# myshell-ai/OpenVoice

Measured on NVIDIA H100. Metric: audio_seconds_per_second, higher is better.
Workload: dtype f32 (3xFP16 split-precision tensor-core convs with fp32 accumulation, fp32 FFMA elsewhere)

## Files before the change

### include/ovc.h

```cpp
#ifndef OVC_B200_H
#define OVC_B200_H

#include <stddef.h>
#include <stdint.h>

#ifdef __cplusplus
extern "C" {
#endif

#define OVC_ABI_VERSION 17

#if defined(__GNUC__)
#define OVC_API __attribute__((visibility("default")))
#else
#define OVC_API
#endif

enum {
  OVC_OK = 0,
  OVC_ERR_INVALID = -1,
  OVC_ERR_CUDA = -2,
  OVC_ERR_STATE = -3,
  OVC_ERR_MISSING = -4,
  OVC_ERR_NOMEM = -5
};
// ... 154 lines not shown
                                      float* d_stats, int32_t* d_cum, float* d_g, int64_t* d_y_lengths, void* stream);
OVC_API int ovc_tts_decode_windows_tokens(ovc_ctx* ctx, const float* stats, const int32_t* cum, const float* g,
                                          const int64_t* y_lengths, int N, int T, const int64_t* row, const int64_t* frame0,
                                          const int64_t* len, int W, int Wmax, const uint64_t* seed, const int64_t* stream,
                                          const float* noise_scale, float* o, float* z_p, void* cuda_stream);

OVC_API int ovc_set_precision(ovc_ctx* ctx, int mode);

#define OVC_OPT_TTS_SIMPLE 2
#define OVC_OPT_GRAPH 3
#define OVC_OPT_PDL 5
#define OVC_OPT_BRANCHES 7
#define OVC_OPT_PAIR 8
#define OVC_OPT_PAIR_OCC 9
#define OVC_OPT_STAGED_EPI 10
OVC_API int ovc_set_option(ovc_ctx* ctx, int key, int value);

OVC_API int ovc_last_launch_count(const ovc_ctx* ctx);

OVC_API int ovc_graph_replays(const ovc_ctx* ctx);

OVC_API int ovc_profile_enable(ovc_ctx* ctx, int enable);
OVC_API int ovc_profile_read(ovc_ctx* ctx, double* ms, int64_t* launches, double* flops, double* bytes);
OVC_API int ovc_profile_detail(ovc_ctx* ctx, int max, char* names, double* ms, double* flops, double* bytes,
                               int* family);

OVC_API int ovc_debug_enable(ovc_ctx* ctx, int enable);
OVC_API int ovc_debug_fetch(ovc_ctx* ctx, const char* name, float* host_out, size_t max_floats,
                    int64_t* shape4 );

// ... 5 lines not shown
```

### openvoice_b200/_native.py

```python
from __future__ import annotations

import ctypes as C
import os
from typing import Dict, Iterable, Optional, Tuple

_HERE = os.path.dirname(os.path.abspath(__file__))
LIB_PATH = os.path.join(_HERE, "libovc_b200.so")

ABI_VERSION = 17
EXPORTS = (
    "ovc_abi_version", "ovc_last_error", "ovc_create", "ovc_destroy", "ovc_load_tensor",
    "ovc_finalize_weights", "ovc_workspace_floats", "ovc_voice_conversion", "ovc_last_launch_count",
    "ovc_profile_enable", "ovc_profile_read", "ovc_profile_detail", "ovc_debug_enable", "ovc_debug_fetch",
    "ovc_spectrogram", "ovc_convert_waveform", "ovc_set_precision", "ovc_reference_encoder",
    "ovc_tts_info", "ovc_tts_encode", "ovc_tts_decode", "ovc_set_option", "ovc_graph_replays",
    "ovc_reference_encoder_ragged", "ovc_resample", "ovc_resample_span", "ovc_voice_conversion_items",
    "ovc_convert_waveform_items", "ovc_tts_encode_items", "ovc_tts_decode_items", "ovc_philox_normals",
    "ovc_tts_encode_state", "ovc_tts_decode_windows", "ovc_spectrogram_ring", "ovc_splice",
    "ovc_tts_encode_state_rows", "ovc_tts_state_rows", "ovc_resample_plan", "ovc_resample_rings",
    "ovc_voice_conversion_frames", "ovc_convert_waveform_frames", "ovc_tone_track_expand",
    "ovc_tts_encode_g", "ovc_tts_encode_state_tokens", "ovc_tts_decode_windows_tokens", "ovc_tts_encode_state_rows_tokens",
    "ovc_tts_state_rows_tokens", "ovc_reference_encoder_stream", "ovc_reference_encoder_stream_state_floats",
    "ovc_generate_frames",
)
# ... 259 lines not shown
            _check(self.lib, rc, f"ovc_load_tensor({k})")
            (ignored if rc == 1 else used).append(k)
        self.finalized = False
        return used, ignored

    def finalize(self):
        _check(self.lib, self.lib.ovc_finalize_weights(self.handle), "ovc_finalize_weights")
        self.finalized = True

    def set_precision(self, mode: str):
        m = PRECISIONS[mode]
        _check(self.lib, self.lib.ovc_set_precision(self.handle, m), "ovc_set_precision")
        self.precision = mode

    def set_option(self, key: str, value: int):
        k = {"tts_simple": 2, "graph": 3, "pdl": 5, "branches": 7, "pair": 8, "pair_occ": 9, "staged_epi": 10}[key]
        _check(self.lib, self.lib.ovc_set_option(self.handle, k, int(value)), "ovc_set_option")

    def voice_conversion(self, spec, lengths, g_src, g_tgt, noise=None, tau: float = 0.3, seed: int = 0,
                         ragged: bool = False, latents: bool = True, stream=None, items: Optional[dict] = None, out=None):
        import torch
        assert spec.is_cuda and spec.dtype == torch.float32 and spec.is_contiguous()
        assert lengths.is_cuda and lengths.dtype == torch.int64 and lengths.is_contiguous()
        B, S, T = spec.shape
        gs, fs = se_arg(g_src, B, self.hp.gin_channels, T, "g_src")
        gt, ft = se_arg(g_tgt, B, self.hp.gin_channels, T, "g_tgt")
        if noise is not None:
            noise = noise.contiguous().float()
            assert tuple(noise.shape) == (B, self.hp.inter_channels, T)
        hop = self.hp.hop_length
        if out is not None:
# ... 486 lines not shown
```

### openvoice_b200/csrc/ovc_lib.cu

```cuda
#include <cuda_runtime.h>

#include <algorithm>
#include <cmath>
#include <cstdarg>
#include <cstdio>
#include <cstdlib>
#include <cstring>
#include <map>
#include <string>
#include <vector>

#include "../../include/ovc.h"
#include "ovc_convpack.h"
#include "ovc_small.cuh"
#include "ovc_tcconv.cuh"
#include "ovc_tts.cuh"
#include "ovc_refenc.cuh"
#include "ovc_resample.cuh"
#include "ovc_splice.h"
#include "ovc_variants.h"

namespace ovc {

static thread_local std::string g_err;
// ... 135 lines not shown
  WNLayers flow_wn[4];
  ConvLayer dec_pre, dec_ups[4];
  ConvLayer rb_c1[12][3], rb_c2[12][3];
  TcLayer tc_c1[12][3], tc_c2[12][3], tc_ups[4], tc_pre;
  float* d_tcw = nullptr;
  std::vector<float> h_tcw;
  int precision = 0;
  bool tts_simple = false;
  bool use_graph = true;
  int use_pdl = 2;
  bool use_branches = true;
  int par_frames = 512;
  bool use_pair = true;
  bool use_pair_occ = true;
  bool use_staged_epi = true;
  bool pair_occ2_ok[TCN_N_OCC2] = {};
  cudaStream_t br_stream[2] = {nullptr, nullptr};
  cudaEvent_t br_ev[4] = {nullptr, nullptr, nullptr, nullptr};
  size_t post_w_off = 0;
  size_t cond_w_off = 0, cond_b_off = 0;
  int* d_cond_wrow = nullptr;
  int* d_cond_sel = nullptr;
  int cond_rows_out = 0;
  int cond_off_enc = 0, cond_off_fsrc = 0, cond_off_ftgt = 0, cond_off_dec = 0;
  int cond_off_enc_tc = 0, cond_off_fsrc_tc = 0, cond_off_ftgt_tc = 0;
  int* d_cond_cols[2][3] = {};
  int cond_pf_cols[2][3] = {};
  int cond_pf_off[2][3][4] = {};

  float2* d_tw = nullptr;
// ... 427 lines not shown
  if (c->d_w) { cudaFree(c->d_w); c->d_w = nullptr; }
  c->w_floats = c->h_w.size();
  CK(cudaMalloc(&c->d_w, c->w_floats * sizeof(float)));
  CK(cudaMemcpy(c->d_w, c->h_w.data(), c->w_floats * sizeof(float), cudaMemcpyHostToDevice));
  if (c->d_tcw) { cudaFree(c->d_tcw); c->d_tcw = nullptr; }
  CK(cudaMalloc(&c->d_tcw, c->h_tcw.size() * sizeof(float)));
  CK(cudaMemcpy(c->d_tcw, c->h_tcw.data(), c->h_tcw.size() * sizeof(float), cudaMemcpyHostToDevice));
  c->h_tcw.clear();
  c->h_tcw.shrink_to_fit();
  for (int TN : {128, 64, 32})
    for (bool staged : {false, true}) {
      const TcKernel k = tc_conv_kernel(TN, staged), p = tc_pair_kernel(TN, TcPairOcc(), staged);
      CK(cudaFuncSetAttribute(k.fn, cudaFuncAttributeMaxDynamicSharedMemorySize, (int)k.smem));
      CK(cudaFuncSetAttribute(p.fn, cudaFuncAttributeMaxDynamicSharedMemorySize, (int)p.smem));
    }
  for (int i = 0; i < TCN_N_OCC2; ++i) {
    const TcKernel k = tc_pair_kernel(kTcPairOcc2[i].C, kTcPairOcc2[i].o);
    CK(cudaFuncSetAttribute(k.fn, cudaFuncAttributeMaxDynamicSharedMemorySize, (int)k.smem));
    int blocks = 0;
    CK(cudaOccupancyMaxActiveBlocksPerMultiprocessor(&blocks, k.fn, k.threads, k.smem));
    c->pair_occ2_ok[i] = blocks >= 2;
    if (blocks < 2)
      fprintf(stderr, "ovc: the C = %d conv-pair kernel with %d operand buffer(s) fits %d CTA(s) per SM, not 2; its pairs run "
              "one CTA per SM\n", kTcPairOcc2[i].C, kTcPairOcc2[i].o.nabuf, blocks);
  }
  if (c->d_cond_wrow) cudaFree(c->d_cond_wrow);
  if (c->d_cond_sel) cudaFree(c->d_cond_sel);
  CK(cudaMalloc(&c->d_cond_wrow, wrow.size() * sizeof(int)));
  CK(cudaMalloc(&c->d_cond_sel, sel.size() * sizeof(int)));
  CK(cudaMemcpy(c->d_cond_wrow, wrow.data(), wrow.size() * sizeof(int), cudaMemcpyHostToDevice));
// ... 135 lines not shown
  CK(cudaEventRecord(c->ev[c->ev_used], r.st));
  return OVC_OK;
}
static int prof_end(Run& r, int variant, int family, double flops, double bytes, int tag = 0) {
  ovc_ctx* c = r.c;
  if (!c->prof) return OVC_OK;
  CK(cudaEventRecord(c->ev[c->ev_used + 1], r.st));
  c->ev_used += 2;
  c->ev_flops.push_back(flops);
  c->ev_bytes.push_back(bytes);
  c->ev_variant.push_back(variant);
  c->ev_family.push_back(family);
  c->ev_tag.push_back(tag);
  return OVC_OK;
}
enum { V_TCPAIR128 = -14, V_TCPAIR64 = -12, V_TCPAIR32 = -13, V_TC128 = -1, V_TC64 = -2, V_TC32 = -3, V_TRANSPOSE = -4, V_TTS_DENSE = -5, V_TTS_LN = -6, V_TTS_SCORES = -7,
       V_TTS_ATTN = -8, V_TTS_DW = -9, V_TTS_SPLINE = -10, V_TTS_MISC = -11 };
static const char* variant_name(int v) {
  if (v >= 0) return kInfo[v].name;
  switch (v) {
    case V_TCPAIR128: return "PAIR_N128";
    case V_TCPAIR64: return "PAIR_N64";
    case V_TCPAIR32: return "PAIR_N32";
    case V_TC128: return "TC3_N128";
    case V_TC64: return "TC3_N64";
    case V_TC32: return "TC3_N32";
    case V_TTS_DENSE: return "TTS_DENSE32";
    case V_TTS_LN: return "TTS_LAYERNORM";
    case V_TTS_SCORES: return "TTS_SCORES";
    case V_TTS_ATTN: return "TTS_ATTN_OUT";
    case V_TTS_DW: return "TTS_DWCONV";
    case V_TTS_SPLINE: return "TTS_SPLINE";
    case V_TTS_MISC: return "TTS_MISC";
    default: return "TRANSPOSE";
  }
}

// ... 58 lines not shown
}

static int launch_pair(Run& r, const TcLayer& T1, const TcLayer& T2, const float* x, float* y, int t_len, int mul, float slope,
                       float scale, int accumulate) {
  TcConvArgs a{};
  const int C = T1.TN;
  a.x = x; a.x_bs = (long long)C * r.P * mul;
  a.w = reinterpret_cast<const uint16_t*>(r.c->d_tcw + T1.w_off);
  a.w2 = reinterpret_cast<const uint16_t*>(r.c->d_tcw + T2.w_off);
  a.bias = r.c->d_tcw + T1.b_off; a.bias2 = r.c->d_tcw + T2.b_off;
  a.y = y; a.y_bs = a.x_bs; a.y_ld = C;
  a.lens = r.glens; a.tmax = r.Tmax; a.mul = mul;
  a.Cin = C; a.Ntot = C; a.K = T1.K; a.DIL = T1.DIL;
  a.slope = slope; a.scale = scale; a.accumulate = accumulate;
  a.passes = r.c->precision == 2 ? 1 : 3;
  TcPairOcc o = r.c->use_pair_occ ? tc_pair_occ(T1, T2) : TcPairOcc();
  for (int i = 0; i < TCN_N_OCC2; ++i)
    if (o.occ == 2 && kTcPairOcc2[i].C == C && kTcPairOcc2[i].o.nabuf == o.nabuf && !r.c->pair_occ2_ok[i]) o = TcPairOcc();
  const TcKernel k = tc_pair_kernel(C, o, r.c->use_staged_epi && tc_stage_pays(T1.K, a.passes));
  if (!k.fn) return fail(OVC_ERR_INVALID, "no conv-pair kernel for C = %d at %d CTA(s) per SM, %d operand buffer(s)", C, o.occ, o.nabuf);
  const TcGrid g = tc_pair_grid(t_len, r.B, T1.K, r.c->sm_count, o.occ);
  const int n_tt = g.n_tt, total = g.total;
  TRY(prof_begin(r));
  dim3 pg((unsigned)g.grid_x, 1, 1);
  CK(launch_ex(k.fn, pg, k.threads, k.smem, r.st, false, a, n_tt, total));
  CK(cudaGetLastError());
  r.c->launches++;
  const double units = (double)r.B * t_len;
  TRY(prof_end(r, C == 128 ? V_TCPAIR128 : C == 64 ? V_TCPAIR64 : V_TCPAIR32, 1, 2.0 * 2.0 * C * C * T1.K * units, 4.0 * C * (2 + (accumulate ? 1 : 0)) * units,
               (C << 16) | (T1.K << 8) | T1.DIL));
  return OVC_OK;
}

static int launch_transpose(Run& r, const float* src, float* dst, int rows, int cols) {
  dim3 grid((cols + 31) / 32, (rows + 31) / 32, r.B);
  TRY(prof_begin(r));
  transpose_kernel<<<grid, 256, 0, r.st>>>(src, dst, rows, cols, (long long)rows * cols);
  CK(cudaGetLastError());
  r.c->launches++;
  TRY(prof_end(r, V_TRANSPOSE, 0, 0.0, 8.0 * rows * cols * r.B));
  return OVC_OK;
}

struct CondRef {
// ... 154 lines not shown
  }
  e->launches = c->launches;
  CK(cudaGraphLaunch(e->exec, st));
  c->graph_replays++;
  return OVC_OK;
}

static int set_call_params(ovc_ctx* c, uint64_t seed, float tau, const ItemParams& items, cudaStream_t st) {
  if (!c->d_callp) CK(cudaMalloc(&c->d_callp, sizeof(CallParams)));
  set_call_params_kernel<<<1, 1, 0, st>>>(c->d_callp, seed, tau, items);
  CK(cudaGetLastError());
  return OVC_OK;
}
static uintptr_t option_bits(const ovc_ctx* c) {
  return (uintptr_t)c->precision | ((uintptr_t)c->use_pdl << 15) | ((uintptr_t)c->use_branches << 14) | ((uintptr_t)c->use_pair << 17) |
         ((uintptr_t)c->use_pair_occ << 18) | ((uintptr_t)c->use_staged_epi << 19);
}

static int ensure_ws(ovc_ctx* c, const WsLayout& W, int B, int Tmax, cudaStream_t st) {
  if (W.total <= c->ws_floats) return OVC_OK;
  CK(cudaStreamSynchronize(st));
  drop_graphs(c);
  if (c->d_ws) CK(cudaFree(c->d_ws));
  c->d_ws = nullptr;
  c->ws_floats = 0;
  cudaError_t e = cudaMalloc(&c->d_ws, W.total * sizeof(float));
  if (e != cudaSuccess) {
    cudaGetLastError();
    return fail(OVC_ERR_NOMEM, "workspace of %.2f GB for B=%d Tmax=%d does not fit: %s", W.total * 4e-9, B, Tmax,
                cudaGetErrorString(e));
  }
// ... 1095 lines not shown
}

int ovc_set_option(ovc_ctx* c, int key, int value) {
  if (!c) return fail(OVC_ERR_INVALID, "null context");
  switch (key) {
    case OVC_OPT_TTS_SIMPLE: c->tts_simple = value != 0; return OVC_OK;
    case OVC_OPT_GRAPH: c->use_graph = value != 0; return OVC_OK;
    case OVC_OPT_PDL:
      if (value < 0 || value > 2) return fail(OVC_ERR_INVALID, "pdl must be 0, 1 or 2");
      c->use_pdl = value;
      return OVC_OK;
    case OVC_OPT_BRANCHES: c->use_branches = value != 0; return OVC_OK;
    case OVC_OPT_PAIR: c->use_pair = value != 0; return OVC_OK;
    case OVC_OPT_PAIR_OCC: c->use_pair_occ = value != 0; return OVC_OK;
    case OVC_OPT_STAGED_EPI: c->use_staged_epi = value != 0; return OVC_OK;
    default: return fail(OVC_ERR_INVALID, "unknown option %d", key);
  }
}

int ovc_last_launch_count(const ovc_ctx* c) { return c ? c->launches : 0; }

int ovc_graph_replays(const ovc_ctx* c) { return c ? c->graph_replays : 0; }

int ovc_profile_enable(ovc_ctx* c, int enable) {
  if (!c) return fail(OVC_ERR_INVALID, "null context");
  c->prof = enable != 0;
  c->ev_used = 0;
  c->ev_flops.clear();
  c->ev_bytes.clear();
  c->ev_variant.clear();
// ... 26 lines not shown
  c->ev_family.clear();
  c->ev_tag.clear();
  return OVC_OK;
}

int ovc_profile_detail(ovc_ctx* c, int max, char* names , double* ms, double* flops, double* bytes, int* family) {
  if (!c) return fail(OVC_ERR_INVALID, "null context");
  int n = 0;
  for (size_t i = 0; i + 1 < c->ev_used && n < max; i += 2, ++n) {
    float m = 0;
    CK(cudaEventElapsedTime(&m, c->ev[i], c->ev[i + 1]));
    if (names) {
      const int tag = c->ev_tag[i / 2], v = c->ev_variant[i / 2];
      if (tag && v == V_TCPAIR128) snprintf(names + 16 * n, 16, "T128Pk%dd%d", (tag >> 8) & 255, tag & 255);
      else if (tag && (v == V_TCPAIR64 || v == V_TCPAIR32)) snprintf(names + 16 * n, 16, "P%dk%dd%d", tag >> 16, (tag >> 8) & 255, tag & 255);
      else if (tag) snprintf(names + 16 * n, 16, "T%dc%dk%dd%d", v == V_TC128 ? 128 : v == V_TC64 ? 64 : 32, tag >> 16, (tag >> 8) & 255, tag & 255);
      else { strncpy(names + 16 * n, variant_name(v), 15); names[16 * n + 15] = 0; }
    }
    if (ms) ms[n] = m;
    if (flops) flops[n] = c->ev_flops[i / 2];
    if (bytes) bytes[n] = c->ev_bytes[i / 2];
    if (family) family[n] = c->ev_family[i / 2];
  }
  return n;
}

int ovc_debug_enable(ovc_ctx* c, int enable) {
  if (!c) return fail(OVC_ERR_INVALID, "null context");
  c->debug = enable != 0;
  return OVC_OK;
// ... 20 lines not shown
```

### openvoice_b200/csrc/ovc_tc.cuh

```cuda
#pragma once
#include <cuda_fp16.h>
#include <cuda_runtime.h>
#include <stdint.h>

namespace ovc {
namespace tc {

__device__ __forceinline__ uint32_t smem_addr(const void* p) { return static_cast<uint32_t>(__cvta_generic_to_shared(p)); }

__device__ __forceinline__ uint64_t make_desc(uint32_t saddr, uint32_t lbo_bytes, uint32_t sbo_bytes) {
  return (uint64_t)((saddr >> 4) & 0x3FFF) | ((uint64_t)((lbo_bytes >> 4) & 0x3FFF) << 16) |
         ((uint64_t)((sbo_bytes >> 4) & 0x3FFF) << 32);
}

template <int N> struct Wgmma;
template <> struct Wgmma<32> {
  static __device__ __forceinline__ void mma(float (&d)[16], uint64_t a, uint64_t b, int scale_d) {
    asm volatile(
        "{\n\t.reg .pred p;\n\tsetp.ne.b32 p, %18, 0;\n\t"
        "wgmma.mma_async.sync.aligned.m64n32k16.f32.f16.f16 {%0, %1, %2, %3, %4, %5, %6, %7, %8, %9, %10, %11, %12, %13, %14, %15}, %16, %17, p, 1, 1, 0, 0;\n\t}"
        : "+f"(d[0]), "+f"(d[1]), "+f"(d[2]), "+f"(d[3]), "+f"(d[4]), "+f"(d[5]), "+f"(d[6]), "+f"(d[7]), "+f"(d[8]), "+f"(d[9]), "+f"(d[10]), "+f"(d[11]), "+f"(d[12]), "+f"(d[13]), "+f"(d[14]), "+f"(d[15])
        : "l"(a), "l"(b), "r"(scale_d));
  }
};
// ... 23 lines not shown
        : "+f"(d[0]), "+f"(d[1]), "+f"(d[2]), "+f"(d[3]), "+f"(d[4]), "+f"(d[5]), "+f"(d[6]), "+f"(d[7]), "+f"(d[8]), "+f"(d[9]), "+f"(d[10]), "+f"(d[11]), "+f"(d[12]), "+f"(d[13]), "+f"(d[14]), "+f"(d[15]), "+f"(d[16]), "+f"(d[17]), "+f"(d[18]), "+f"(d[19]), "+f"(d[20]), "+f"(d[21]), "+f"(d[22]), "+f"(d[23]), "+f"(d[24]), "+f"(d[25]), "+f"(d[26]), "+f"(d[27]), "+f"(d[28]), "+f"(d[29]), "+f"(d[30]), "+f"(d[31]), "+f"(d[32]), "+f"(d[33]), "+f"(d[34]), "+f"(d[35]), "+f"(d[36]), "+f"(d[37]), "+f"(d[38]), "+f"(d[39]), "+f"(d[40]), "+f"(d[41]), "+f"(d[42]), "+f"(d[43]), "+f"(d[44]), "+f"(d[45]), "+f"(d[46]), "+f"(d[47]), "+f"(d[48]), "+f"(d[49]), "+f"(d[50]), "+f"(d[51]), "+f"(d[52]), "+f"(d[53]), "+f"(d[54]), "+f"(d[55]), "+f"(d[56]), "+f"(d[57]), "+f"(d[58]), "+f"(d[59]), "+f"(d[60]), "+f"(d[61]), "+f"(d[62]), "+f"(d[63]), "+f"(d[64]), "+f"(d[65]), "+f"(d[66]), "+f"(d[67]), "+f"(d[68]), "+f"(d[69]), "+f"(d[70]), "+f"(d[71]), "+f"(d[72]), "+f"(d[73]), "+f"(d[74]), "+f"(d[75]), "+f"(d[76]), "+f"(d[77]), "+f"(d[78]), "+f"(d[79]), "+f"(d[80]), "+f"(d[81]), "+f"(d[82]), "+f"(d[83]), "+f"(d[84]), "+f"(d[85]), "+f"(d[86]), "+f"(d[87]), "+f"(d[88]), "+f"(d[89]), "+f"(d[90]), "+f"(d[91]), "+f"(d[92]), "+f"(d[93]), "+f"(d[94]), "+f"(d[95]), "+f"(d[96]), "+f"(d[97]), "+f"(d[98]), "+f"(d[99]), "+f"(d[100]), "+f"(d[101]), "+f"(d[102]), "+f"(d[103]), "+f"(d[104]), "+f"(d[105]), "+f"(d[106]), "+f"(d[107]), "+f"(d[108]), "+f"(d[109]), "+f"(d[110]), "+f"(d[111]), "+f"(d[112]), "+f"(d[113]), "+f"(d[114]), "+f"(d[115]), "+f"(d[116]), "+f"(d[117]), "+f"(d[118]), "+f"(d[119]), "+f"(d[120]), "+f"(d[121]), "+f"(d[122]), "+f"(d[123]), "+f"(d[124]), "+f"(d[125]), "+f"(d[126]), "+f"(d[127])
        : "l"(a), "l"(b), "r"(scale_d));
  }
};

__device__ __forceinline__ void wgmma_fence() { asm volatile("wgmma.fence.sync.aligned;" ::: "memory"); }
__device__ __forceinline__ void wgmma_commit() { asm volatile("wgmma.commit_group.sync.aligned;" ::: "memory"); }
template <int N>
__device__ __forceinline__ void wgmma_wait() { asm volatile("wgmma.wait_group.sync.aligned %0;" ::"n"(N) : "memory"); }
template <int R>
__device__ __forceinline__ void fence_regs(float (&d)[R]) {
#pragma unroll
  for (int i = 0; i < R; ++i) asm volatile("" : "+f"(d[i])::"memory");
}

template <int R> __device__ __forceinline__ void regs_dealloc() { asm volatile("setmaxnreg.dec.sync.aligned.u32 %0;" ::"n"(R)); }
template <int R> __device__ __forceinline__ void regs_alloc() { asm volatile("setmaxnreg.inc.sync.aligned.u32 %0;" ::"n"(R)); }

constexpr float kLoScale = 2048.f, kLoInv = 1.f / 2048.f;

__device__ __forceinline__ void split_f16x8(float4 a, float4 b, float slope, uint4& hi, uint4& lo) {
  float x[8] = {a.x, a.y, a.z, a.w, b.x, b.y, b.z, b.w};
  uint32_t h[4], l[4];
#pragma unroll
  for (int i = 0; i < 4; ++i) {
    float x0 = x[2 * i], x1 = x[2 * i + 1];
    x0 = fmaxf(x0, x0 * slope);
    x1 = fmaxf(x1, x1 * slope);
    const __half2 hh = __floats2half2_rn(x0, x1);
    const float2 hf = __half22float2(hh);
// ... 11 lines not shown
```

### openvoice_b200/csrc/ovc_tcconv.cuh

```cuda
#pragma once
#include "ovc_conv.cuh"
#include "ovc_tc.cuh"
#include "ovc_tcpack.h"

namespace ovc {

struct TcConvArgs {
  const float* x; long long x_bs;
  const uint16_t* w;
  const float* bias; long long bias_bs;
  float* y; long long y_bs; int y_ld;
  const float* r;
  float* s; long long s_bs;
  int epi;
  int split; int first;
  const long long* lens; int tmax; int mul;
  const long long* lens_x; int has_lens_x;
  int Cin; int Ntot; int K; int DIL;
  float slope; float scale; int accumulate;
  int passes;
  const uint16_t* w2; const float* bias2;
  long long bias_ts;
};

// ... 97 lines not shown
  if (a.bias_ts) tc_epilogue_body<TN, true>(a, v_at, b, t0, n0, lim, row_a);
  else tc_epilogue_body<TN, false>(a, v_at, b, t0, n0, lim, row_a);
}

template <int TN>
__device__ __forceinline__ void tc_epilogue(const TcConvArgs& a, const float (&d)[TN], int b, int t0, int n0, int lim, int row_a) {
  const bool two = a.passes == 3;
  tc_epilogue_v<TN>(a, [&](int j) { return tc_result<TN>(d, two, j); }, b, t0, n0, lim, row_a);
}
__device__ __forceinline__ TcConvArgs tc_pair_epilogue_args(const TcConvArgs& a, int TN) {
  TcConvArgs e = a;
  e.y_ld = TN; e.r = a.x; e.bias = a.bias2; e.bias_bs = 0; e.bias_ts = 0; e.epi = 0;
  return e;
}

template <int TN>
__device__ __forceinline__ void tc_mma_step(float (&d)[TN], uint64_t a_hi, uint64_t a_lo, uint64_t b, bool three, bool first) {
  float (&lo)[TN / 2] = *reinterpret_cast<float(*)[TN / 2]>(&d[TN / 2]);
  float (&hi)[TN / 2] = *reinterpret_cast<float(*)[TN / 2]>(&d[0]);
  tc::Wgmma<TN>::mma(hi, a_hi, b, first ? 0 : 1);
  if (three) {
    tc::Wgmma<TN>::mma(lo, a_hi, b + TN, first ? 0 : 1);
    tc::Wgmma<TN>::mma(lo, a_lo, b, 1);
  }
}

constexpr int TCN_THREADS = 384;
constexpr int TCN_NCT = 96;

template <int TN, bool PAIR, int OCC = 1, int NAB = 2, bool STAGED = false>
struct TcnCfg {
  static_assert(!PAIR || TN == 32 || TN == 64 || TN == 128, "conv pairs: C = 32, 64 or 128");
  static_assert(OCC == 1 || (PAIR && TN <= 64), "two CTAs per SM: C = 32 / 64 pairs");
  static_assert(!STAGED || (TN == 128 && OCC == 1), "staged epilogue: TN = 128, one CTA per SM");
  static constexpr int THREADS = STAGED ? TCN_THREADS + 128 : TCN_THREADS;
  static constexpr int KCH = 32, NKC = KCH / 8;
  static constexpr int ROWS = 194;
  static constexpr int ROWS2 = TCN_ROWS2;
  static constexpr int NABUF = NAB;
  static constexpr int RING = PAIR ? tc_pair_ring(TN, OCC, NAB) : tc_ring_slots(TN, PAIR);
  static constexpr int SLOT_BYTES = 2 * 2 * TN * 16;
  static constexpr int A_BUF_BYTES = 2 * NKC * ROWS * 16;
  static constexpr int A2_BYTES = PAIR ? 2 * (TN / 8) * ROWS2 * 16 : 0;
  static constexpr int STAGE_BYTES = STAGED ? (TN / 2) * 256 * 4 : 0;
  static_assert(!STAGED || !PAIR || STAGE_BYTES <= A2_BYTES, "a pair's staging tile lies in its conv-2 operand");
  static constexpr int SBUF_BYTES = STAGED && !PAIR ? STAGE_BYTES : 0;
  static constexpr size_t SMEM_BYTES = 1024 + NABUF * A_BUF_BYTES + A2_BYTES + RING * SLOT_BYTES + SBUF_BYTES;
  static_assert(!PAIR || SMEM_BYTES == tc_pair_smem(TN, NABUF, RING), "tc_pair_smem");
  static_assert(SMEM_BYTES <= (OCC == 1 ? 232448 : TCN_SMEM_OCC2), "shared memory budget");
  static_assert((2 * NABUF + 2 * RING + 2) * 8 <= 1024, "barrier area");
  static constexpr int PROD_REGS = OCC == 1 && !STAGED ? 56 : 32, MMA_REGS = STAGED ? 184 : OCC == 1 ? 224 : 104;
  static constexpr int STORE_REGS = 112;
  static_assert(128 * PROD_REGS + 256 * MMA_REGS + (STAGED ? 128 * STORE_REGS : 0) <= 65536 / OCC, "register budget");
};

template <int TN, bool PAIR, int OCC = 1, int NAB = 2, bool STAGED = false>
__global__ void __launch_bounds__(TcnCfg<TN, PAIR, OCC, NAB, STAGED>::THREADS, OCC) tcconv_kernel(const TcConvArgs a, int n_tt, int total) {
  using Cfg = TcnCfg<TN, PAIR, OCC, NAB, STAGED>;
  constexpr int ROWS = Cfg::ROWS, ROWS2 = Cfg::ROWS2, NABUF = Cfg::NABUF, RING = Cfg::RING, NKC = Cfg::NKC;
  extern __shared__ __align__(128) unsigned char smem_raw[];
  uint64_t* bars = reinterpret_cast<uint64_t*>(smem_raw);
  uint64_t *a_full = bars, *a_empty = bars + NABUF, *b_full = a_empty + NABUF, *b_empty = b_full + RING;
  uint64_t *s_full = b_empty + RING, *s_empty = s_full + 1;
  unsigned char* abuf = smem_raw + 1024;
  unsigned char* a2buf = abuf + NABUF * Cfg::A_BUF_BYTES;
  unsigned char* bring = a2buf + Cfg::A2_BYTES;
  float* stage = reinterpret_cast<float*>(PAIR ? a2buf : bring + RING * Cfg::SLOT_BYTES);

  const int tid = threadIdx.x, lane = tid & 31;
  const int warp = __shfl_sync(0xffffffffu, tid >> 5, 0);
  const int H1 = (a.K - 1) / 2 * a.DIL;
  const int H2 = PAIR ? (a.K - 1) / 2 : 0;
  const int R = 128 - 2 * H2;
  const int rows8 = (128 + 2 * H1 + 7) & ~7;
  const int nq = a.Cin / Cfg::KCH;
  const int n_slots = (a.Cin / 16) * a.K;
  const int n_w = PAIR ? 2 * n_slots : n_slots;
  const bool resident = n_w <= RING;
  if (H1 > TCN_HMAX || (PAIR && 128 + 2 * H2 > ROWS2)) __trap();
  constexpr uint32_t BYTES = Cfg::SLOT_BYTES;

  if (tid == 0) {
    for (int i = 0; i < NABUF; ++i) { mbar_init(&a_full[i], TCN_NCT); mbar_init(&a_empty[i], 2); }
    for (int i = 0; i < RING; ++i) { mbar_init(&b_full[i], 1); mbar_init(&b_empty[i], 2); }
    if (STAGED) { mbar_init(s_full, 256); mbar_init(s_empty, 128); }
    fence_mbar_init();
  }
  if (PAIR) {
    for (int i = tid; i < Cfg::A2_BYTES / 16; i += Cfg::THREADS) reinterpret_cast<uint4*>(a2buf)[i] = make_uint4(0u, 0u, 0u, 0u);
    asm volatile("fence.proxy.async.shared::cta;" ::: "memory");
  }
  __syncthreads();
  pdl_launch_dependents();
  if (warp != 0) pdl_wait();
// ... 81 lines not shown
      }
    }
  } else if (STAGED && warp >= 12) {
    tc::regs_dealloc<Cfg::STORE_REGS>();
    const int st = tid & 127;
    uint32_t phase = 0;
    TCN_FOR_TILES
      if (PAIR) named_bar_arrive(1, 384);
      mbar_wait(s_full, phase);
      phase ^= 1;
#pragma unroll 1
      for (int h = 0; h < 2; ++h) {
        const float* sv = stage + h * 128 + st;
        const auto v_at = [&](int j) { return sv[j * 256]; };
        const int row_a = 64 * h + 16 * (warp & 3) + (lane >> 2);
        if constexpr (PAIR) tc_epilogue_v<TN>(tc_pair_epilogue_args(a, TN), v_at, b, t0, 0, min(lim, t0 + R), row_a);
        else tc_epilogue_v<TN>(a, v_at, b, t0, blockIdx.y * TN, lim, row_a);
      }
      if (!PAIR) mbar_arrive(s_empty);
    }
  } else {
    tc::regs_alloc<Cfg::MMA_REGS>();
    const int wg = (warp >> 2) - 1;
    const bool leader = (tid & 127) == 0;
    const int row_a = 64 * wg + 16 * (warp & 3) + (lane >> 2);
    constexpr uint32_t LBO_A = ROWS * 16, LBO_A2 = ROWS2 * 16, LBO_B = 2 * TN * 16, SBO = 128;
    constexpr uint32_t A_LO16 = (NKC * ROWS * 16) >> 4, A2_LO16 = ((TN / 8) * ROWS2 * 16) >> 4, SLOT16 = BYTES >> 4;
    const uint64_t a_proto = tc::make_desc(0, LBO_A, SBO), b_proto = tc::make_desc(0, LBO_B, SBO);
    const uint64_t b_ring = b_proto + (tc::smem_addr(bring) >> 4);
    const bool three = a.passes == 3;
    float d[TN];
#pragma unroll
    for (int i = 0; i < TN; ++i) d[i] = 0.f;
    const auto stage_tile = [&]() {
// ... 110 lines not shown
        } else {
          tc_epilogue<TN>(tc_pair_epilogue_args(a, TN), d, b, t0, 0, min(lim, t0 + R), row_a);
        }
      }
    }
  }
#undef TCN_FOR_TILES
}

struct TcKernel {
  void (*fn)(TcConvArgs, int, int) = nullptr;
  size_t smem = 0;
  int threads = 0;
};
using TcPairKernel = TcKernel;
template <int TN, bool PAIR, int OCC = 1, int NAB = 2, bool STAGED = false>
inline TcKernel tc_kernel() {
  using Cfg = TcnCfg<TN, PAIR, OCC, NAB, STAGED>;
  return {tcconv_kernel<TN, PAIR, OCC, NAB, STAGED>, Cfg::SMEM_BYTES, Cfg::THREADS};
}
inline bool tc_stage_pays(int K, int passes) { return passes * K >= 15; }
inline TcKernel tc_conv_kernel(int TN, bool staged) {
  if (TN == 128) return staged ? tc_kernel<128, false, 1, 2, true>() : tc_kernel<128, false>();
  if (TN == 64) return tc_kernel<64, false>();
  if (TN == 32) return tc_kernel<32, false>();
  return {};
}
inline TcKernel tc_pair_kernel(int C, TcPairOcc o, bool staged = false) {
  if (o.occ == 1 && o.nabuf == 2) {
    if (C == 128) return staged ? tc_kernel<128, true, 1, 2, true>() : tc_kernel<128, true>();
    if (C == 64) return tc_kernel<64, true>();
    if (C == 32) return tc_kernel<32, true>();
  } else if (o.occ == 2) {
    if (C == 32 && o.nabuf == 2) return tc_kernel<32, true, 2, 2>();
    if (C == 32 && o.nabuf == 1) return tc_kernel<32, true, 2, 1>();
    if (C == 64 && o.nabuf == 1) return tc_kernel<64, true, 2, 1>();
  }
  return {};
}
constexpr int TCN_N_OCC2 = 3;
constexpr struct { int C; TcPairOcc o; } kTcPairOcc2[TCN_N_OCC2] = {{32, {2, 2}}, {32, {2, 1}}, {64, {2, 1}}};

template <int C>
__global__ void __launch_bounds__(256) conv_post_cl_kernel(const float* __restrict__ x, long long x_bs,
                                                           const float* __restrict__ w, float* __restrict__ y,
                                                           long long y_bs, int y_len, const long long* lens, int tmax,
                                                           int mul) {
  constexpr int TB = 256, ROWS = TB + 6, LD = ROWS + 3;
  __shared__ float ws[7][C];
  __shared__ float xs[C][LD];
  for (int i = threadIdx.x; i < C * 7; i += blockDim.x) ws[i % 7][i / 7] = w[i];
  const int b = blockIdx.y;
  const int lim = (lens ? (int)min((long long)tmax, lens[b]) : tmax) * mul;
// ... 46 lines not shown
```

### openvoice_b200/csrc/ovc_tcpack.h

```cpp
#pragma once
#include <cuda_fp16.h>
#include <stddef.h>
#include <stdint.h>

#include <algorithm>

namespace ovc {

constexpr int TCN_HMAX = 25;
constexpr int TCN_ROWS2 = 146;

constexpr int tc_ring_slots(int TN, bool pair) {
  return pair ? (TN == 32 ? 44 : TN == 64 ? 24 : 12) : (TN == 32 ? 22 : 12);
}

struct TcGeom {
  int Cin = 0, Ntot = 0, K = 0, DIL = 1, TN = 0;
};

inline int tc_tile_n(int Ntot, int Cin, int K, int DIL) {
  if (Ntot <= 0 || Cin <= 0 || K <= 0 || DIL <= 0) return 0;
  if (Ntot % 32 || Cin % 32 || (K - 1) / 2 * DIL > TCN_HMAX) return 0;
  return Ntot % 128 == 0 ? 128 : (Ntot % 64 == 0 ? 64 : 32);
}
// ... 84 lines not shown
}

struct TcPairOcc {
  int occ = 1, nabuf = 2;
};
inline TcPairOcc tc_pair_occ(const TcGeom& T1, const TcGeom& T2) {
  TcPairOcc o;
  if (!tc_pair_fuses(T1, T2)) return o;
  const int n_w = 2 * (T1.Cin / 16) * T1.K;
  if (T1.TN == 32 && n_w <= tc_pair_ring(32, 2, 2)) o = {2, 2};
  else if (T1.TN == 32 && n_w <= tc_pair_ring(32, 2, 1)) o = {2, 1};
  else if (T1.TN == 64 && n_w > tc_pair_ring(64, 1, 2)) o = {2, 1};
  return o;
}

}
```

Baseline: 2394.

## Add time-on-N conv-pair kernel for C=64 with 256-frame tiles

Adds a conv-pair variant for 64-channel resblock pairs that maps weights to the wgmma A operand and time to the N dimension. Each CTA then covers 256 frames instead of 128, so the halo overhead per tile shrinks and each MMA instruction is wider. The intermediate activation is written back to shared memory with stmatrix.trans. The variant is on by default and also gets its own staged-epilogue threshold. The trade-offs are more register and shared-memory pressure, one CTA per SM instead of two, and fewer tiles for small inputs, which could hurt load balance.

```diff
diff --git a/include/ovc.h b/include/ovc.h
--- a/include/ovc.h
+++ b/include/ovc.h
@@ -8,7 +8,7 @@
 extern "C" {
 #endif
 
-#define OVC_ABI_VERSION 17
+#define OVC_ABI_VERSION 18
 
 #if defined(__GNUC__)
 #define OVC_API __attribute__((visibility("default")))
@@ -193,6 +193,7 @@
 #define OVC_OPT_PAIR 8
 #define OVC_OPT_PAIR_OCC 9
 #define OVC_OPT_STAGED_EPI 10
+#define OVC_OPT_PAIR_TN 11
 OVC_API int ovc_set_option(ovc_ctx* ctx, int key, int value);
 
 OVC_API int ovc_last_launch_count(const ovc_ctx* ctx);
diff --git a/openvoice_b200/_native.py b/openvoice_b200/_native.py
--- a/openvoice_b200/_native.py
+++ b/openvoice_b200/_native.py
@@ -7,7 +7,7 @@
 _HERE = os.path.dirname(os.path.abspath(__file__))
 LIB_PATH = os.path.join(_HERE, "libovc_b200.so")
 
-ABI_VERSION = 17
+ABI_VERSION = 18
 EXPORTS = (
     "ovc_abi_version", "ovc_last_error", "ovc_create", "ovc_destroy", "ovc_load_tensor",
     "ovc_finalize_weights", "ovc_workspace_floats", "ovc_voice_conversion", "ovc_last_launch_count",
@@ -297,7 +297,7 @@
         self.precision = mode
 
     def set_option(self, key: str, value: int):
-        k = {"tts_simple": 2, "graph": 3, "pdl": 5, "branches": 7, "pair": 8, "pair_occ": 9, "staged_epi": 10}[key]
+        k = {"tts_simple": 2, "graph": 3, "pdl": 5, "branches": 7, "pair": 8, "pair_occ": 9, "staged_epi": 10, "pair_tn": 11}[key]
         _check(self.lib, self.lib.ovc_set_option(self.handle, k, int(value)), "ovc_set_option")
 
     def voice_conversion(self, spec, lengths, g_src, g_tgt, noise=None, tau: float = 0.3, seed: int = 0,
diff --git a/openvoice_b200/csrc/ovc_lib.cu b/openvoice_b200/csrc/ovc_lib.cu
--- a/openvoice_b200/csrc/ovc_lib.cu
+++ b/openvoice_b200/csrc/ovc_lib.cu
@@ -173,6 +173,7 @@
   bool use_pair = true;
   bool use_pair_occ = true;
   bool use_staged_epi = true;
+  bool use_pair_tn = true;
   bool pair_occ2_ok[TCN_N_OCC2] = {};
   cudaStream_t br_stream[2] = {nullptr, nullptr};
   cudaEvent_t br_ev[4] = {nullptr, nullptr, nullptr, nullptr};
@@ -630,6 +631,10 @@
       CK(cudaFuncSetAttribute(k.fn, cudaFuncAttributeMaxDynamicSharedMemorySize, (int)k.smem));
       CK(cudaFuncSetAttribute(p.fn, cudaFuncAttributeMaxDynamicSharedMemorySize, (int)p.smem));
     }
+  for (bool staged : {false, true}) {
+    const TcKernel k = tc_pair_tn_kernel(staged);
+    CK(cudaFuncSetAttribute(k.fn, cudaFuncAttributeMaxDynamicSharedMemorySize, (int)k.smem));
+  }
   for (int i = 0; i < TCN_N_OCC2; ++i) {
     const TcKernel k = tc_pair_kernel(kTcPairOcc2[i].C, kTcPairOcc2[i].o);
     CK(cudaFuncSetAttribute(k.fn, cudaFuncAttributeMaxDynamicSharedMemorySize, (int)k.smem));
@@ -795,13 +800,14 @@
   c->ev_tag.push_back(tag);
   return OVC_OK;
 }
-enum { V_TCPAIR128 = -14, V_TCPAIR64 = -12, V_TCPAIR32 = -13, V_TC128 = -1, V_TC64 = -2, V_TC32 = -3, V_TRANSPOSE = -4, V_TTS_DENSE = -5, V_TTS_LN = -6, V_TTS_SCORES = -7,
+enum { V_TCPAIR128 = -14, V_TCPAIR64 = -12, V_TCPAIR32 = -13, V_TCPAIR64TN = -15, V_TC128 = -1, V_TC64 = -2, V_TC32 = -3, V_TRANSPOSE = -4, V_TTS_DENSE = -5, V_TTS_LN = -6, V_TTS_SCORES = -7,
        V_TTS_ATTN = -8, V_TTS_DW = -9, V_TTS_SPLINE = -10, V_TTS_MISC = -11 };
 static const char* variant_name(int v) {
   if (v >= 0) return kInfo[v].name;
   switch (v) {
     case V_TCPAIR128: return "PAIR_N128";
     case V_TCPAIR64: return "PAIR_N64";
+    case V_TCPAIR64TN: return "PAIR_N64_TN";
     case V_TCPAIR32: return "PAIR_N32";
     case V_TC128: return "TC3_N128";
     case V_TC64: return "TC3_N64";
@@ -890,12 +896,13 @@
   a.Cin = C; a.Ntot = C; a.K = T1.K; a.DIL = T1.DIL;
   a.slope = slope; a.scale = scale; a.accumulate = accumulate;
   a.passes = r.c->precision == 2 ? 1 : 3;
-  TcPairOcc o = r.c->use_pair_occ ? tc_pair_occ(T1, T2) : TcPairOcc();
+  const bool tn = r.c->use_pair_tn && tc_pair_tn(T1, T2);
+  TcPairOcc o = r.c->use_pair_occ && !tn ? tc_pair_occ(T1, T2) : TcPairOcc();
   for (int i = 0; i < TCN_N_OCC2; ++i)
     if (o.occ == 2 && kTcPairOcc2[i].C == C && kTcPairOcc2[i].o.nabuf == o.nabuf && !r.c->pair_occ2_ok[i]) o = TcPairOcc();
-  const TcKernel k = tc_pair_kernel(C, o, r.c->use_staged_epi && tc_stage_pays(T1.K, a.passes));
+  const TcKernel k = tn ? tc_pair_tn_kernel(r.c->use_staged_epi && tc_pair_tn_staged(T1.K, a.passes)) : tc_pair_kernel(C, o, r.c->use_staged_epi && tc_stage_pays(T1.K, a.passes));
   if (!k.fn) return fail(OVC_ERR_INVALID, "no conv-pair kernel for C = %d at %d CTA(s) per SM, %d operand buffer(s)", C, o.occ, o.nabuf);
-  const TcGrid g = tc_pair_grid(t_len, r.B, T1.K, r.c->sm_count, o.occ);
+  const TcGrid g = tn ? tc_pair_tn_grid(t_len, r.B, T1.K, r.c->sm_count) : tc_pair_grid(t_len, r.B, T1.K, r.c->sm_count, o.occ);
   const int n_tt = g.n_tt, total = g.total;
   TRY(prof_begin(r));
   dim3 pg((unsigned)g.grid_x, 1, 1);
@@ -903,7 +910,7 @@
   CK(cudaGetLastError());
   r.c->launches++;
   const double units = (double)r.B * t_len;
-  TRY(prof_end(r, C == 128 ? V_TCPAIR128 : C == 64 ? V_TCPAIR64 : V_TCPAIR32, 1, 2.0 * 2.0 * C * C * T1.K * units, 4.0 * C * (2 + (accumulate ? 1 : 0)) * units,
+  TRY(prof_end(r, tn ? V_TCPAIR64TN : C == 128 ? V_TCPAIR128 : C == 64 ? V_TCPAIR64 : V_TCPAIR32, 1, 2.0 * 2.0 * C * C * T1.K * units, 4.0 * C * (2 + (accumulate ? 1 : 0)) * units,
                (C << 16) | (T1.K << 8) | T1.DIL));
   return OVC_OK;
 }
@@ -1088,7 +1095,7 @@
 }
 static uintptr_t option_bits(const ovc_ctx* c) {
   return (uintptr_t)c->precision | ((uintptr_t)c->use_pdl << 15) | ((uintptr_t)c->use_branches << 14) | ((uintptr_t)c->use_pair << 17) |
-         ((uintptr_t)c->use_pair_occ << 18) | ((uintptr_t)c->use_staged_epi << 19);
+         ((uintptr_t)c->use_pair_occ << 18) | ((uintptr_t)c->use_staged_epi << 19) | ((uintptr_t)c->use_pair_tn << 20);
 }
 
 static int ensure_ws(ovc_ctx* c, const WsLayout& W, int B, int Tmax, cudaStream_t st) {
@@ -2214,6 +2221,7 @@
     case OVC_OPT_PAIR: c->use_pair = value != 0; return OVC_OK;
     case OVC_OPT_PAIR_OCC: c->use_pair_occ = value != 0; return OVC_OK;
     case OVC_OPT_STAGED_EPI: c->use_staged_epi = value != 0; return OVC_OK;
+    case OVC_OPT_PAIR_TN: c->use_pair_tn = value != 0; return OVC_OK;
     default: return fail(OVC_ERR_INVALID, "unknown option %d", key);
   }
 }
@@ -2270,6 +2278,7 @@
       const int tag = c->ev_tag[i / 2], v = c->ev_variant[i / 2];
       if (tag && v == V_TCPAIR128) snprintf(names + 16 * n, 16, "T128Pk%dd%d", (tag >> 8) & 255, tag & 255);
       else if (tag && (v == V_TCPAIR64 || v == V_TCPAIR32)) snprintf(names + 16 * n, 16, "P%dk%dd%d", tag >> 16, (tag >> 8) & 255, tag & 255);
+      else if (tag && v == V_TCPAIR64TN) snprintf(names + 16 * n, 16, "P%dTk%dd%d", tag >> 16, (tag >> 8) & 255, tag & 255);
       else if (tag) snprintf(names + 16 * n, 16, "T%dc%dk%dd%d", v == V_TC128 ? 128 : v == V_TC64 ? 64 : 32, tag >> 16, (tag >> 8) & 255, tag & 255);
       else { strncpy(names + 16 * n, variant_name(v), 15); names[16 * n + 15] = 0; }
     }
diff --git a/openvoice_b200/csrc/ovc_tc.cuh b/openvoice_b200/csrc/ovc_tc.cuh
--- a/openvoice_b200/csrc/ovc_tc.cuh
+++ b/openvoice_b200/csrc/ovc_tc.cuh
@@ -61,6 +61,11 @@
   for (int i = 0; i < R; ++i) asm volatile("" : "+f"(d[i])::"memory");
 }
 
+__device__ __forceinline__ void stmatrix_x4_trans(uint32_t addr, const uint32_t (&r)[4]) {
+  asm volatile("stmatrix.sync.aligned.m8n8.x4.trans.shared.b16 [%0], {%1, %2, %3, %4};" ::"r"(addr), "r"(r[0]), "r"(r[1]), "r"(r[2]), "r"(r[3])
+               : "memory");
+}
+
 template <int R> __device__ __forceinline__ void regs_dealloc() { asm volatile("setmaxnreg.dec.sync.aligned.u32 %0;" ::"n"(R)); }
 template <int R> __device__ __forceinline__ void regs_alloc() { asm volatile("setmaxnreg.inc.sync.aligned.u32 %0;" ::"n"(R)); }
 
diff --git a/openvoice_b200/csrc/ovc_tcconv.cuh b/openvoice_b200/csrc/ovc_tcconv.cuh
--- a/openvoice_b200/csrc/ovc_tcconv.cuh
+++ b/openvoice_b200/csrc/ovc_tcconv.cuh
@@ -135,6 +135,34 @@
   return e;
 }
 
+template <int TN, int GC, class V>
+__device__ __forceinline__ void tc_pair_tn_epilogue(const TcConvArgs& a, V v_at, int b, int t0, int lim2, int n_a, int c_a) {
+  const float b2a = __ldg(a.bias2 + n_a), b2b = __ldg(a.bias2 + n_a + 8);
+  const float* rb = a.x + (size_t)b * a.y_bs;
+  float* yb = a.y + (size_t)b * a.y_bs;
+#pragma unroll
+  for (int g0 = 0; g0 < TN / 4; g0 += GC) {
+    float rv[4 * GC], yv[4 * GC];
+#pragma unroll
+    for (int e = 0; e < 4 * GC; ++e) {
+      const int t = t0 + c_a + 8 * (g0 + e / 4) + (e & 1), n = n_a + (e & 2) * 4;
+      const bool ok = t < lim2;
+      const size_t off = (size_t)t * TN + n;
+      rv[e] = ok ? rb[off] : 0.f;
+      yv[e] = ok && a.accumulate ? yb[off] : 0.f;
+    }
+#pragma unroll
+    for (int e = 0; e < 4 * GC; ++e) {
+      const int t = t0 + c_a + 8 * (g0 + e / 4) + (e & 1), n = n_a + (e & 2) * 4;
+      float o = v_at(4 * g0 + e) + ((e & 2) ? b2b : b2a);
+      o += rv[e];
+      if (a.accumulate) o = yv[e] + o;
+      if (a.scale != 1.f) o *= a.scale;
+      if (t < lim2) yb[(size_t)t * TN + n] = o;
+    }
+  }
+}
+
 template <int TN>
 __device__ __forceinline__ void tc_mma_step(float (&d)[TN], uint64_t a_hi, uint64_t a_lo, uint64_t b, bool three, bool first) {
   float (&lo)[TN / 2] = *reinterpret_cast<float(*)[TN / 2]>(&d[TN / 2]);
@@ -146,28 +174,41 @@
   }
 }
 
+__device__ __forceinline__ void tc_mma_step_tn(float (&d)[128], uint64_t w, uint64_t x_hi, uint64_t x_lo, bool three, bool first) {
+  float (&lo)[64] = *reinterpret_cast<float(*)[64]>(&d[64]);
+  float (&hi)[64] = *reinterpret_cast<float(*)[64]>(&d[0]);
+  tc::Wgmma<128>::mma(hi, w, x_hi, first ? 0 : 1);
+  if (three) {
+    tc::Wgmma<128>::mma(lo, w + ((64 * 16) >> 4), x_hi, first ? 0 : 1);
+    tc::Wgmma<128>::mma(lo, w, x_lo, 1);
+  }
+}
+
 constexpr int TCN_THREADS = 384;
 constexpr int TCN_NCT = 96;
 
-template <int TN, bool PAIR, int OCC = 1, int NAB = 2, bool STAGED = false>
+template <int TN, bool PAIR, int OCC = 1, int NAB = 2, bool STAGED = false, bool TT = false>
 struct TcnCfg {
   static_assert(!PAIR || TN == 32 || TN == 64 || TN == 128, "conv pairs: C = 32, 64 or 128");
   static_assert(OCC == 1 || (PAIR && TN <= 64), "two CTAs per SM: C = 32 / 64 pairs");
-  static_assert(!STAGED || (TN == 128 && OCC == 1), "staged epilogue: TN = 128, one CTA per SM");
+  static_assert(!STAGED || ((TN == 128 || TT) && OCC == 1), "staged epilogue: TN = 128 or time on N, one CTA per SM");
+  static_assert(!TT || (PAIR && TN == 64 && OCC == 1), "time on N: C = 64 pairs, one CTA per SM");
   static constexpr int THREADS = STAGED ? TCN_THREADS + 128 : TCN_THREADS;
   static constexpr int KCH = 32, NKC = KCH / 8;
-  static constexpr int ROWS = 194;
-  static constexpr int ROWS2 = TCN_ROWS2;
+  static constexpr int TILE = TT ? TCN_TN_TILE : 128;
+  static constexpr int ROWS = TT ? TCN_TN_ROWS : 194;
+  static constexpr int ROWS2 = TT ? TCN_TN_ROWS2 : TCN_ROWS2;
+  static_assert(ROWS % 8 == 2 && ROWS2 % 8 == 2 && ROWS >= ((TILE + 2 * TCN_HMAX + 7) & ~7), "operand pitches");
   static constexpr int NABUF = NAB;
-  static constexpr int RING = PAIR ? tc_pair_ring(TN, OCC, NAB) : tc_ring_slots(TN, PAIR);
+  static constexpr int RING = TT ? tc_pair_tn_ring(NAB) : PAIR ? tc_pair_ring(TN, OCC, NAB) : tc_ring_slots(TN, PAIR);
   static constexpr int SLOT_BYTES = 2 * 2 * TN * 16;
   static constexpr int A_BUF_BYTES = 2 * NKC * ROWS * 16;
   static constexpr int A2_BYTES = PAIR ? 2 * (TN / 8) * ROWS2 * 16 : 0;
-  static constexpr int STAGE_BYTES = STAGED ? (TN / 2) * 256 * 4 : 0;
+  static constexpr int STAGE_BYTES = STAGED ? (TT ? TN : TN / 2) * 256 * 4 : 0;
   static_assert(!STAGED || !PAIR || STAGE_BYTES <= A2_BYTES, "a pair's staging tile lies in its conv-2 operand");
   static constexpr int SBUF_BYTES = STAGED && !PAIR ? STAGE_BYTES : 0;
   static constexpr size_t SMEM_BYTES = 1024 + NABUF * A_BUF_BYTES + A2_BYTES + RING * SLOT_BYTES + SBUF_BYTES;
-  static_assert(!PAIR || SMEM_BYTES == tc_pair_smem(TN, NABUF, RING), "tc_pair_smem");
+  static_assert(!PAIR || SMEM_BYTES == (TT ? tc_pair_tn_smem(NABUF, RING) : tc_pair_smem(TN, NABUF, RING)), "tc_pair_smem");
   static_assert(SMEM_BYTES <= (OCC == 1 ? 232448 : TCN_SMEM_OCC2), "shared memory budget");
   static_assert((2 * NABUF + 2 * RING + 2) * 8 <= 1024, "barrier area");
   static constexpr int PROD_REGS = OCC == 1 && !STAGED ? 56 : 32, MMA_REGS = STAGED ? 184 : OCC == 1 ? 224 : 104;
@@ -175,9 +216,9 @@
   static_assert(128 * PROD_REGS + 256 * MMA_REGS + (STAGED ? 128 * STORE_REGS : 0) <= 65536 / OCC, "register budget");
 };
 
-template <int TN, bool PAIR, int OCC = 1, int NAB = 2, bool STAGED = false>
-__global__ void __launch_bounds__(TcnCfg<TN, PAIR, OCC, NAB, STAGED>::THREADS, OCC) tcconv_kernel(const TcConvArgs a, int n_tt, int total) {
-  using Cfg = TcnCfg<TN, PAIR, OCC, NAB, STAGED>;
+template <int TN, bool PAIR, int OCC = 1, int NAB = 2, bool STAGED = false, bool TT = false>
+__global__ void __launch_bounds__(TcnCfg<TN, PAIR, OCC, NAB, STAGED, TT>::THREADS, OCC) tcconv_kernel(const TcConvArgs a, int n_tt, int total) {
+  using Cfg = TcnCfg<TN, PAIR, OCC, NAB, STAGED, TT>;
   constexpr int ROWS = Cfg::ROWS, ROWS2 = Cfg::ROWS2, NABUF = Cfg::NABUF, RING = Cfg::RING, NKC = Cfg::NKC;
   extern __shared__ __align__(128) unsigned char smem_raw[];
   uint64_t* bars = reinterpret_cast<uint64_t*>(smem_raw);
@@ -192,13 +233,13 @@
   const int warp = __shfl_sync(0xffffffffu, tid >> 5, 0);
   const int H1 = (a.K - 1) / 2 * a.DIL;
   const int H2 = PAIR ? (a.K - 1) / 2 : 0;
-  const int R = 128 - 2 * H2;
-  const int rows8 = (128 + 2 * H1 + 7) & ~7;
+  const int R = Cfg::TILE - 2 * H2;
+  const int rows8 = (Cfg::TILE + 2 * H1 + 7) & ~7;
   const int nq = a.Cin / Cfg::KCH;
   const int n_slots = (a.Cin / 16) * a.K;
   const int n_w = PAIR ? 2 * n_slots : n_slots;
   const bool resident = n_w <= RING;
-  if (H1 > TCN_HMAX || (PAIR && 128 + 2 * H2 > ROWS2)) __trap();
+  if (H1 > TCN_HMAX || (PAIR && Cfg::TILE + 2 * H2 > ROWS2)) __trap();
   constexpr uint32_t BYTES = Cfg::SLOT_BYTES;
 
   if (tid == 0) {
@@ -310,10 +351,136 @@
         const float* sv = stage + h * 128 + st;
         const auto v_at = [&](int j) { return sv[j * 256]; };
         const int row_a = 64 * h + 16 * (warp & 3) + (lane >> 2);
-        if constexpr (PAIR) tc_epilogue_v<TN>(tc_pair_epilogue_args(a, TN), v_at, b, t0, 0, min(lim, t0 + R), row_a);
+        if constexpr (TT) tc_pair_tn_epilogue<TN, 4>(a, v_at, b, t0, min(lim, t0 + R), 16 * (warp & 3) + (lane >> 2), 128 * h + 2 * (lane & 3));
+        else if constexpr (PAIR) tc_epilogue_v<TN>(tc_pair_epilogue_args(a, TN), v_at, b, t0, 0, min(lim, t0 + R), row_a);
         else tc_epilogue_v<TN>(a, v_at, b, t0, blockIdx.y * TN, lim, row_a);
       }
       if (!PAIR) mbar_arrive(s_empty);
+    }
+  } else if constexpr (TT) {
+    tc::regs_alloc<Cfg::MMA_REGS>();
+    const int wg = (warp >> 2) - 1;
+    const bool leader = (tid & 127) == 0;
+    const int n_a = 16 * (warp & 3) + (lane >> 2);
+    const int c_a = 128 * wg + 2 * (lane & 3);
+    constexpr uint32_t LBO_X = ROWS * 16, LBO_X2 = ROWS2 * 16, LBO_W = 2 * TN * 16, SBO = 128;
+    constexpr uint32_t X_LO16 = (NKC * ROWS * 16) >> 4, X2_LO16 = ((TN / 8) * ROWS2 * 16) >> 4, SLOT16 = BYTES >> 4;
+    const uint64_t x_proto = tc::make_desc(0, LBO_X, SBO), w_proto = tc::make_desc(0, LBO_W, SBO);
+    const uint64_t w_ring = w_proto + (tc::smem_addr(bring) >> 4);
+    const bool three = a.passes == 3;
+    float d[2 * TN];
+#pragma unroll
+    for (int i = 0; i < 2 * TN; ++i) d[i] = 0.f;
+    if (resident)
+      for (int it = 0; it < n_w; ++it) mbar_wait(&b_full[it], 0u);
+    int slot = 0, buf = 0;
+    uint32_t bphase = 0, aphase = 0;
+    TCN_FOR_TILES
+      bool first = true;
+      if (resident) slot = 0;
+      for (int q = 0; q < nq; ++q) {
+        mbar_wait(&a_full[buf], aphase);
+        tc::fence_regs(d);
+        tc::wgmma_fence();
+        int prev = -1;
+        for (int j = 0; j < 2; ++j) {
+          uint64_t x_cur = x_proto + ((tc::smem_addr(abuf + buf * Cfg::A_BUF_BYTES) + 128 * wg * 16 + 2 * j * LBO_X) >> 4);
+          for (int tap = 0; tap < a.K; ++tap) {
+            if (!resident) mbar_wait(&b_full[slot], bphase);
+            tc_mma_step_tn(d, w_ring + (uint32_t)slot * SLOT16, x_cur, x_cur + X_LO16, three, first);
+            tc::wgmma_commit();
+            if (!resident) {
+              tc::wgmma_wait<1>();
+              if (leader && prev >= 0) mbar_arrive(&b_empty[prev]);
+              prev = slot;
+            }
+            first = false;
+            x_cur += a.DIL;
+            if (++slot == RING) { slot = 0; bphase ^= 1; }
+          }
+        }
+        tc::wgmma_wait<0>();
+        tc::fence_regs(d);
+        if (leader) {
+          if (prev >= 0) mbar_arrive(&b_empty[prev]);
+          mbar_arrive(&a_empty[buf]);
+        }
+        if (++buf == NABUF) { buf = 0; aphase ^= 1; }
+      }
+      named_bar_sync(1, STAGED ? 384 : 256);
+      {
+        const float bias_a = __ldg(a.bias + n_a), bias_b = __ldg(a.bias + n_a + 8);
+        const int mi = lane >> 3;
+        const uint32_t st_row = tc::smem_addr(a2buf) +
+                                (((2 * (warp & 3) + (mi & 1)) * ROWS2 + 128 * wg + 8 * (mi >> 1) + (lane & 7)) * 16);
+        constexpr uint32_t A2_LO = (TN / 8) * ROWS2 * 16;
+#pragma unroll
+        for (int g = 0; g < TN / 4; g += 2) {
+          uint32_t h[4], l[4];
+#pragma unroll
+          for (int u = 0; u < 2; ++u) {
+            float x[4];
+#pragma unroll
+            for (int i = 0; i < 4; ++i)
+              x[i] = (three ? fmaf(d[TN + 4 * (g + u) + i], tc::kLoInv, d[4 * (g + u) + i]) : d[4 * (g + u) + i]) + (i < 2 ? bias_a : bias_b);
+            const int t = t0 - H2 + c_a + 8 * (g + u);
+            const bool ok0 = t >= 0 && t < lim, ok1 = t + 1 >= 0 && t + 1 < lim;
+            x[0] = ok0 ? fmaxf(x[0], x[0] * a.slope) : 0.f;
+            x[1] = ok1 ? fmaxf(x[1], x[1] * a.slope) : 0.f;
+            x[2] = ok0 ? fmaxf(x[2], x[2] * a.slope) : 0.f;
+            x[3] = ok1 ? fmaxf(x[3], x[3] * a.slope) : 0.f;
+            const __half2 ha = __floats2half2_rn(x[0], x[1]), hb = __floats2half2_rn(x[2], x[3]);
+            const float2 fa = __half22float2(ha), fb = __half22float2(hb);
+            const __half2 la = __floats2half2_rn((x[0] - fa.x) * tc::kLoScale, (x[1] - fa.y) * tc::kLoScale);
+            const __half2 lb = __floats2half2_rn((x[2] - fb.x) * tc::kLoScale, (x[3] - fb.y) * tc::kLoScale);
+            h[2 * u] = *reinterpret_cast<const uint32_t*>(&ha);
+            h[2 * u + 1] = *reinterpret_cast<const uint32_t*>(&hb);
+            l[2 * u] = *reinterpret_cast<const uint32_t*>(&la);
+            l[2 * u + 1] = *reinterpret_cast<const uint32_t*>(&lb);
+          }
+          tc::stmatrix_x4_trans(st_row + 8 * g * 16, h);
+          tc::stmatrix_x4_trans(st_row + A2_LO + 8 * g * 16, l);
+        }
+      }
+      asm volatile("fence.proxy.async.shared::cta;" ::: "memory");
+      named_bar_sync(2, 256);
+      {
+        const uint64_t x2_proto = tc::make_desc(0, LBO_X2, SBO);
+        tc::fence_regs(d);
+        tc::wgmma_fence();
+        bool first2 = true;
+        int prev = -1;
+        for (int kk = 0; kk < TN / 16; ++kk) {
+          uint64_t x_cur = x2_proto + ((tc::smem_addr(a2buf) + 128 * wg * 16 + 2 * kk * LBO_X2) >> 4);
+          for (int tap = 0; tap < a.K; ++tap) {
+            if (resident) {
+              tc_mma_step_tn(d, w_ring + (uint32_t)(n_slots + kk * a.K + tap) * SLOT16, x_cur, x_cur + X2_LO16, three, first2);
+            } else {
+              mbar_wait(&b_full[slot], bphase);
+              tc_mma_step_tn(d, w_ring + (uint32_t)slot * SLOT16, x_cur, x_cur + X2_LO16, three, first2);
+              tc::wgmma_commit();
+              tc::wgmma_wait<1>();
+              if (leader && prev >= 0) mbar_arrive(&b_empty[prev]);
+              prev = slot;
+              if (++slot == RING) { slot = 0; bphase ^= 1; }
+            }
+            first2 = false;
+            x_cur += 1;
+          }
+        }
+        tc::wgmma_commit();
+        tc::wgmma_wait<0>();
+        tc::fence_regs(d);
+        if (leader && prev >= 0) mbar_arrive(&b_empty[prev]);
+      }
+      if constexpr (STAGED) {
+        named_bar_sync(3, 256);
+#pragma unroll
+        for (int j = 0; j < TN; ++j) stage[j * 256 + tid - 128] = tc_result<2 * TN>(d, three, j);
+        mbar_arrive(s_full);
+      } else {
+        tc_pair_tn_epilogue<TN, 8>(a, [&](int j) { return tc_result<2 * TN>(d, three, j); }, b, t0, min(lim, t0 + R), n_a, c_a);
+      }
     }
   } else {
     tc::regs_alloc<Cfg::MMA_REGS>();
@@ -454,10 +621,10 @@
   int threads = 0;
 };
 using TcPairKernel = TcKernel;
-template <int TN, bool PAIR, int OCC = 1, int NAB = 2, bool STAGED = false>
+template <int TN, bool PAIR, int OCC = 1, int NAB = 2, bool STAGED = false, bool TT = false>
 inline TcKernel tc_kernel() {
-  using Cfg = TcnCfg<TN, PAIR, OCC, NAB, STAGED>;
-  return {tcconv_kernel<TN, PAIR, OCC, NAB, STAGED>, Cfg::SMEM_BYTES, Cfg::THREADS};
+  using Cfg = TcnCfg<TN, PAIR, OCC, NAB, STAGED, TT>;
+  return {tcconv_kernel<TN, PAIR, OCC, NAB, STAGED, TT>, Cfg::SMEM_BYTES, Cfg::THREADS};
 }
 inline bool tc_stage_pays(int K, int passes) { return passes * K >= 15; }
 inline TcKernel tc_conv_kernel(int TN, bool staged) {
@@ -477,6 +644,9 @@
     if (C == 64 && o.nabuf == 1) return tc_kernel<64, true, 2, 1>();
   }
   return {};
+}
+inline TcKernel tc_pair_tn_kernel(bool staged) {
+  return staged ? tc_kernel<64, true, 1, TCN_TN_NAB, true, true>() : tc_kernel<64, true, 1, TCN_TN_NAB, false, true>();
 }
 constexpr int TCN_N_OCC2 = 3;
 constexpr struct { int C; TcPairOcc o; } kTcPairOcc2[TCN_N_OCC2] = {{32, {2, 2}}, {32, {2, 1}}, {64, {2, 1}}};
diff --git a/openvoice_b200/csrc/ovc_tcpack.h b/openvoice_b200/csrc/ovc_tcpack.h
--- a/openvoice_b200/csrc/ovc_tcpack.h
+++ b/openvoice_b200/csrc/ovc_tcpack.h
@@ -122,4 +122,27 @@
   return o;
 }
 
+constexpr int TCN_TN_TILE = 256;
+constexpr int TCN_TN_ROWS = 314;
+constexpr int TCN_TN_ROWS2 = 266;
+constexpr size_t tc_pair_tn_smem(int nabuf, int ring) {
+  return 1024 + (size_t)nabuf * 2 * 4 * TCN_TN_ROWS * 16 + (size_t)2 * 8 * TCN_TN_ROWS2 * 16 + (size_t)ring * 2 * 2 * 64 * 16;
 }
+constexpr int tc_pair_tn_ring(int nabuf) { return (int)((232448 - tc_pair_tn_smem(nabuf, 0)) / (2 * 2 * 64 * 16)); }
+
+inline bool tc_pair_tn(const TcGeom& T1, const TcGeom& T2) {
+  return tc_pair_fuses(T1, T2) && T1.TN == 64 && TCN_TN_TILE + 2 * ((T2.K - 1) / 2) <= TCN_TN_ROWS2;
+}
+inline bool tc_pair_tn_staged(int K, int passes) { return passes * K >= 11; }
+constexpr int TCN_TN_NAB = 2;
+inline TcGrid tc_pair_tn_grid(int t_len, int B, int K, int sm_count) {
+  TcGrid g;
+  const int R = TCN_TN_TILE - (K - 1);
+  g.n_tt = (t_len + R - 1) / R;
+  g.total = g.n_tt * B;
+  g.ncol = 1;
+  g.grid_x = std::min(g.total, sm_count);
+  return g;
+}
+
+}
```

After: 2471, median of 6. +3.2%, better.
